# imazen/codec-eval

Hardware: AMD Instinct MI355X
Metric: metric MP/s (SSIMULACRA2+DSSIM+Butteraugli) at 1/2/4/8 GPU; HBM-roofline % (higher is better)
Workload: dtype f32

## Files before the change

### codec-eval_amd/csrc/butteraugli.hip

```cpp
#include <algorithm>
#include <cmath>
#include <cstdlib>
#include <type_traits>

#include "ba_front_geom.h"
#include "ba_slot_order.h"
#include "ce_internal.h"

namespace {

constexpr int TPB = 256;
constexpr int PSY = 10;
enum { UHF0 = 0, UHF1, HF0, HF1, MF0, MF1, MF2, LF0, LF1, LF2 };

struct blur_kernel {
    int len;
    float k[40];
    float lo[16], hi[16];
};

#define BA_XY                                                           \
    const uint32_t x = blockIdx.x * 64 + (threadIdx.x & 63);            \
    const uint32_t y = blockIdx.y * 4 + (threadIdx.x >> 6);             \
    if (x >= g.w || y >= g.h) return;                                   \
// ... 476 lines not shown
                float v[BW_OUT + LEN - 1];
#pragma unroll
                for (int j = 0; j < BW_OUT + LEN - 1; j++) v[j] = tile[(ly + j) * TW + c];
#pragma unroll
                for (int o = 0; o < BW_OUT; o++) {
                    float sum = 0.0f;
#pragma unroll
                    for (int j = 0; j < LEN; j++) sum = blur_tap(sum, v[o + j], bk.k[j]);
                    res[q][part][o] = sum * border_scale<LEN>(bk, gy0 + o, (int)g.h, inv_wsum);
                }
            }
        }
        if (HV && q + 1 < NP) {
            stash();
            __syncthreads();
        }
    }
    if (!col_live) return;
    const size_t pl = g.plane;
#pragma unroll
    for (int part = 0; part < PARTS; part++) {
        const int gy0 = y0 + 32 * part + 8 * wv;
        if (gy0 >= (int)g.h) break;
        float *ps = psy + (size_t)slot * PSY * g.plane + (size_t)gy0 * g.pitch + gx;
#pragma unroll
        for (int o = 0; o < BW_OUT; o++) {
            if (gy0 + o >= (int)g.h) break;
            float *q = ps + (size_t)o * g.pitch;
            const size_t ao = (size_t)slot * 3 * pl + (size_t)(gy0 + o) * g.pitch + gx;
            if (EPI == EPI_LF) {
                const float *xs = xyb + (size_t)slot * 3 * pl + (size_t)(gy0 + o) * g.pitch + gx;
                const float lx = res[0][part][o], ly = res[1][part][o], lb = res[2][part][o];
                aux_out[ao] = xs[0] - lx;
                aux_out[ao + pl] = xs[pl] - ly;
                aux_out[ao + 2 * pl] = xs[2 * pl] - lb;
                const float xmul = 33.832837186260f, ymul = 14.458268100570f, bmul = 49.87984651440f, y_to_b_mul = -0.362267051518f;
                const float bb = __builtin_fmaf(y_to_b_mul, ly, lb);
                q[LF2 * pl] = bb * bmul;
                q[LF0 * pl] = lx * xmul;
                q[LF1 * pl] = ly * ymul;
            } else if (EPI == EPI_MF) {
                const float kRemoveMfRange = 0.29f, kAddMfRange = 0.1f;
                const float mf0 = res[0][part][o], mf1 = res[1][part][o];
                const float hf0 = tmp[ao] - mf0, hf1 = tmp[ao + pl] - mf1;
                q[MF0 * pl] = remove_range(kRemoveMfRange, mf0);
                q[MF1 * pl] = amplify_range(kAddMfRange, mf1);
                q[MF2 * pl] = res[2][part][o];
                const float suppress = 46.0f, sv = 0.653020556257f, one_minus_s = 1.0f - 0.653020556257f;
                const float scaler = __builtin_fmaf(suppress / __builtin_fmaf(hf1, hf1, suppress), one_minus_s, sv);
                aux_out[ao] = scaler * hf0;
                aux_out[ao + pl] = hf1;
            } else if (EPI == EPI_MASK) {
                aux_out[(size_t)slot * pl + (size_t)(gy0 + o) * g.pitch + gx] = res[0][part][o];
            } else {
                const float kRemoveHfRange = 1.5f, kAddHfRange = 0.132f, kRemoveUhfRange = 0.04f;
                const float kMaxclampHf = 28.4691806922f, kMaxclampUhf = 5.19175294647f, kMulYHf = 2.155f, kMulYUhf = 2.69313763794f;
                float hf0_out, uhf0_out, hf1_out, uhf1_out;
                {
                    const float hf = res[0][part][o];
                    const float uhf = tmp[ao] - hf;
                    hf0_out = remove_range(kRemoveHfRange, hf);
                    uhf0_out = remove_range(kRemoveUhfRange, uhf);
                    q[HF0 * pl] = hf0_out;
                    q[UHF0 * pl] = uhf0_out;
                }
                {
                    float hf = maximum_clamp(res[1][part][o], kMaxclampHf);
                    float uhf = tmp[ao + pl] - hf;
                    uhf = maximum_clamp(uhf, kMaxclampUhf);
                    uhf *= kMulYUhf;
                    uhf1_out = uhf;
                    q[UHF1 * pl] = uhf;
                    hf *= kMulYHf;
                    hf1_out = amplify_range(kAddHfRange, hf);
                    q[HF1 * pl] = hf1_out;
                }
                mask_in[(size_t)slot * pl + (size_t)(gy0 + o) * g.pitch + gx] = mask_pre_one(uhf0_out, hf0_out, uhf1_out, hf1_out);
            }
        }
    }
}

struct malta_params {
    float norm2_0gt1, norm2_0lt1, norm1;
};

struct mline {
    int n;
    signed char d[9][2];
};

__device__ constexpr mline MALTA_HF[16] = {
    {9, {{-4, 0}, {-3, 0}, {-2, 0}, {-1, 0}, {0, 0}, {1, 0}, {2, 0}, {3, 0}, {4, 0}}},
    {9, {{0, -4}, {0, -3}, {0, -2}, {0, -1}, {0, 0}, {0, 1}, {0, 2}, {0, 3}, {0, 4}}},
    {7, {{-3, -3}, {-2, -2}, {-1, -1}, {0, 0}, {1, 1}, {2, 2}, {3, 3}}},
    {7, {{3, -3}, {2, -2}, {1, -1}, {0, 0}, {-1, 1}, {-2, 2}, {-3, 3}}},
    {9, {{1, -4}, {1, -3}, {1, -2}, {0, -1}, {0, 0}, {0, 1}, {-1, 2}, {-1, 3}, {-1, 4}}},
    {9, {{-1, -4}, {-1, -3}, {-1, -2}, {0, -1}, {0, 0}, {0, 1}, {1, 2}, {1, 3}, {1, 4}}},
    {9, {{-4, -1}, {-3, -1}, {-2, -1}, {-1, 0}, {0, 0}, {1, 0}, {2, 1}, {3, 1}, {4, 1}}},
    {9, {{-4, 1}, {-3, 1}, {-2, 1}, {-1, 0}, {0, 0}, {1, 0}, {2, -1}, {3, -1}, {4, -1}}},
    {7, {{-2, -3}, {-1, -2}, {-1, -1}, {0, 0}, {1, 1}, {1, 2}, {2, 3}}},
    {7, {{2, -3}, {1, -2}, {1, -1}, {0, 0}, {-1, 1}, {-1, 2}, {-2, 3}}},
    {7, {{-3, -2}, {-2, -1}, {-1, -1}, {0, 0}, {1, 1}, {2, 1}, {3, 2}}},
    {7, {{3, -2}, {2, -1}, {1, -1}, {0, 0}, {-1, 1}, {-2, 1}, {-3, 2}}},
    {8, {{-4, 2}, {-3, 2}, {-2, 1}, {-1, 1}, {0, 0}, {1, 0}, {2, -1}, {3, -1}}},
    {8, {{-4, -2}, {-3, -2}, {-2, -1}, {-1, -1}, {0, 0}, {1, 0}, {2, 1}, {3, 1}}},
    {8, {{-2, -4}, {-2, -3}, {-1, -2}, {-1, -1}, {0, 0}, {0, 1}, {1, 2}, {1, 3}}},
    {8, {{2, -4}, {2, -3}, {1, -2}, {1, -1}, {0, 0}, {0, 1}, {-1, 2}, {-1, 3}}},
};
__device__ constexpr mline MALTA_LF[16] = {
    {5, {{-4, 0}, {-2, 0}, {0, 0}, {2, 0}, {4, 0}}},
    {5, {{0, -4}, {0, -2}, {0, 0}, {0, 2}, {0, 4}}},
    {5, {{-3, -3}, {-2, -2}, {0, 0}, {2, 2}, {3, 3}}},
    {5, {{3, -3}, {2, -2}, {0, 0}, {-2, 2}, {-3, 3}}},
    {5, {{1, -4}, {1, -2}, {0, 0}, {-1, 2}, {-1, 4}}},
    {5, {{-1, -4}, {-1, -2}, {0, 0}, {1, 2}, {1, 4}}},
    {5, {{-4, -1}, {-2, -1}, {0, 0}, {2, 1}, {4, 1}}},
    {5, {{-4, 1}, {-2, 1}, {0, 0}, {2, -1}, {4, -1}}},
    {5, {{-2, -3}, {-1, -2}, {0, 0}, {1, 2}, {2, 3}}},
    {5, {{2, -3}, {1, -2}, {0, 0}, {-1, 2}, {-2, 3}}},
    {5, {{-3, -2}, {-2, -1}, {0, 0}, {2, 1}, {3, 2}}},
    {5, {{3, -2}, {2, -1}, {0, 0}, {-2, 1}, {-3, 2}}},
    {5, {{-4, 2}, {-2, 1}, {0, 0}, {2, -1}, {4, -2}}},
    {5, {{-4, -2}, {-2, -1}, {0, 0}, {2, 1}, {4, 2}}},
    {5, {{-2, -4}, {-1, -2}, {0, 0}, {1, 2}, {2, 4}}},
    {5, {{2, -4}, {1, -2}, {0, 0}, {-1, 2}, {-2, 4}}},
};

constexpr int MT = 64, MH = 4, ML = MT + 2 * MH;

__device__ constexpr bool malta_line_descends(const mline &ln)
{
    for (int j = 1; j < ln.n; j++)
        if (ln.d[j][1] > ln.d[j - 1][1]) return false;
    return ln.d[0][1] != ln.d[ln.n - 1][1];
}
__device__ constexpr bool malta_line_monotone(const mline &ln)
{
    bool up = true, down = true;
    for (int j = 1; j < ln.n; j++) {
        if (ln.d[j][1] < ln.d[j - 1][1]) up = false;
        if (ln.d[j][1] > ln.d[j - 1][1]) down = false;
    }
    return up || down;
}
__device__ constexpr bool malta_tables_monotone()
{
    for (int k = 0; k < 16; k++)
        if (!malta_line_monotone(MALTA_HF[k]) || !malta_line_monotone(MALTA_LF[k])) return false;
    return true;
}
static_assert(malta_tables_monotone(), "the row-streaming Malta unit needs every line's rows to be visited in one direction");

struct malta_bands {
    malta_params p[2][3];
};

__device__ __forceinline__ void div2_shared_rcp(float a0, float a1, float b, float &q0, float &q1)
{
    const float r = ce_rcp_refined(b);
    q0 = ce_div_refined(a0, b, r);
    q1 = ce_div_refined(a1, b, r);
}

__device__ __forceinline__ float malta_pre_diff(float v0, float v1, const malta_params &mp)
{
    const float absval = 0.5f * (fabsf(v0) + fabsf(v1));
    const float diff = v0 - v1;
    float scaler, scaler2;
    div2_shared_rcp(mp.norm2_0gt1, mp.norm2_0lt1, mp.norm1 + absval, scaler, scaler2);
    const float r = scaler * diff;
    const float fabs0 = fabsf(v0), too_small = 0.55f * fabs0, too_big = 1.05f * fabs0;
    const bool neg = v0 < 0;
    const float u = neg ? -v1 : v1;
    const bool lo = u < too_small, hi = u > too_big;
    const float impact = scaler2 * (lo ? too_small - u : u - too_big);
    const float rn = r + ((neg == lo) ? -impact : impact);
    return (lo || hi) ? rn : r;
}

__device__ __forceinline__ float l2_asym_acc(float total, float val0, float val1, float vw_0gt1, float vw_0lt1)
{
    const float diff = val0 - val1;
    total = __builtin_fmaf(diff * diff, vw_0gt1, total);
    const float fabs0 = fabsf(val0);
    const float too_small = 0.4f * fabs0, too_big = fabs0;
    const float if_neg = val1 > -too_small ? val1 + too_small : (val1 < -too_big ? -val1 - too_big : 0.0f);
    const float if_pos = val1 < too_small ? too_small - val1 : (val1 > too_big ? val1 - too_big : 0.0f);
    const float v = val0 < 0.0f ? if_neg : if_pos;
    return __builtin_fmaf(vw_0lt1, v * v, total);
}

template <bool LF>
__device__ __forceinline__ void malta_rows_xy(const ba_f2 *__restrict__ base, ba_f2 (&acc)[2])
{
    ba_f2 sum[2][16];
    ba_f2 parked[2][16][9];
#pragma unroll
    for (int r = 0; r < 9; r++) {
        ba_f2 v[10];
        const float4 *row = reinterpret_cast<const float4 *>(base + r * ML);
#pragma unroll
        for (int q = 0; q < 5; q++) {
            const float4 t = row[q];
            v[2 * q] = ba_f2{t.x, t.y};
            v[2 * q + 1] = ba_f2{t.z, t.w};
        }
        const int dy = r - 4;
#pragma unroll
        for (int o = 0; o < 2; o++) {
#pragma unroll
            for (int k = 0; k < 16; k++) {
                const mline &ln = LF ? MALTA_LF[k] : MALTA_HF[k];
                if (!malta_line_descends(ln)) {
#pragma unroll
                    for (int j = 0; j < 9; j++)
                        if (j < ln.n && ln.d[j][1] == dy) {
                            const ba_f2 t = v[4 + o + ln.d[j][0]];
                            sum[o][k] = j == 0 ? t : sum[o][k] + t;
                        }
                } else if (dy == ln.d[0][1]) {
                    ba_f2 acc_k = {0.0f, 0.0f};
#pragma unroll
                    for (int j = 0; j < 9; j++)
                        if (j < ln.n) {
                            const ba_f2 t = ln.d[j][1] == dy ? v[4 + o + ln.d[j][0]] : parked[o][k][j];
                            acc_k = j == 0 ? t : acc_k + t;
                        }
                    sum[o][k] = acc_k;
                } else {
#pragma unroll
                    for (int j = 0; j < 9; j++)
                        if (j < ln.n && ln.d[j][1] == dy) parked[o][k][j] = v[4 + o + ln.d[j][0]];
                }
            }
        }
    }
#pragma unroll
    for (int o = 0; o < 2; o++) {
        ba_f2 ret = {0.0f, 0.0f};
#pragma unroll
        for (int k = 0; k < 16; k++) ret = __builtin_elementwise_fma(sum[o][k], sum[o][k], ret);
        acc[o] = acc[o] + ret;
    }
}

template <int MR, int NT, bool FINAL, bool STORE>
__global__ __launch_bounds__(NT, NT == 256 ? 3 : 4) void k_ba_malta_l2_xy(const float *__restrict__ psy, const uint32_t *__restrict__ pair_ref,
                                                           const float *__restrict__ blurred, const float *__restrict__ mask_vals,
                                                           float *__restrict__ diffmap, ce_plane_geom g, uint32_t max_refs,
                                                           malta_bands mb, const uint2 *__restrict__ work, uint32_t tiles_x,
                                                           const float *__restrict__ sub_map, ce_plane_geom gs, int has_sub,
                                                           float *__restrict__ blk_max, double *__restrict__ blk_sums, uint32_t n_blocks)
{
    constexpr int MLR = MR + 2 * MH, RSTEP = NT / 32;
    __shared__ __attribute__((aligned(16))) ba_f2 s[MLR * ML];
    __shared__ __attribute__((aligned(16))) ba_f2 s_acc[MR * MT];
    const uint2 wi = work[blockIdx.x];
    if (wi.x == ~0u) return;
    const uint32_t p = wi.y, bx = wi.x % tiles_x, by = wi.x / tiles_x;
    const int x0 = (int)bx * MT - MH, y0 = (int)by * MR - MH;
    const float *a = psy + (size_t)pair_ref[p] * PSY * g.plane;
    const float *b = psy + (size_t)(max_refs + p) * PSY * g.plane;
    const int tq = threadIdx.x & 31, ty = threadIdx.x >> 5;
    const float wmul[9] = {400.0f, 1.50815703118f, 0.0f, 2150.0f, 10.6195433239f, 16.2176043152f, 29.2353797994f, 0.844626970982f, 0.703646627719f};
    const float hf_asymmetry = 1.0f;
#pragma unroll
    for (int band = 0; band < 3; band++) {
        const malta_params mpx = mb.p[0][band], mpy = mb.p[1][band];
        const uint32_t plane0 = band == 0 ? UHF0 : band == 1 ? HF0 : MF0;
        const float *pax = a + (size_t)plane0 * g.plane, *pbx = b + (size_t)plane0 * g.plane;
        const float *pay = pax + g.plane, *pby = pbx + g.plane;
        for (int i = threadIdx.x; i < MLR * (ML / 4); i += NT) {
            const int ly = i / (ML / 4), lq = i % (ML / 4), gx = x0 + 4 * lq, gy = y0 + ly;
            float4 vax = make_float4(0.f, 0.f, 0.f, 0.f), vbx = vax, vay = vax, vby = vax;
            const bool in = gx >= 0 && gy >= 0 && gx < (int)g.pitch && gy < (int)g.h;
            if (in) {
                const size_t o = (size_t)gy * g.pitch + gx;
                vax = *reinterpret_cast<const float4 *>(pax + o);
                vbx = *reinterpret_cast<const float4 *>(pbx + o);
                vay = *reinterpret_cast<const float4 *>(pay + o);
                vby = *reinterpret_cast<const float4 *>(pby + o);
            }
            const bool i0 = in && gx < (int)g.w, i1 = in && gx + 1 < (int)g.w, i2 = in && gx + 2 < (int)g.w, i3 = in && gx + 3 < (int)g.w;
            float4 r01, r23;
            r01.x = i0 ? malta_pre_diff(vax.x, vbx.x, mpx) : 0.0f;
            r01.y = i0 ? malta_pre_diff(vay.x, vby.x, mpy) : 0.0f;
            r01.z = i1 ? malta_pre_diff(vax.y, vbx.y, mpx) : 0.0f;
            r01.w = i1 ? malta_pre_diff(vay.y, vby.y, mpy) : 0.0f;
            r23.x = i2 ? malta_pre_diff(vax.z, vbx.z, mpx) : 0.0f;
            r23.y = i2 ? malta_pre_diff(vay.z, vby.z, mpy) : 0.0f;
            r23.z = i3 ? malta_pre_diff(vax.w, vbx.w, mpx) : 0.0f;
            r23.w = i3 ? malta_pre_diff(vay.w, vby.w, mpy) : 0.0f;
            float4 *dst = reinterpret_cast<float4 *>(s + ly * ML + 4 * lq);
            dst[0] = r01;
            dst[1] = r23;
            if (band >= 1 && ly >= MH && ly < MH + MR && lq >= MH / 4 && lq < (MH + MT) / 4 && gy < (int)g.h) {
                float4 *pa = reinterpret_cast<float4 *>(s_acc + (ly - MH) * MT + 4 * lq - MH);
                float4 t01 = pa[0], t23 = pa[1];
                if (band == 1) {
                    const float gx_ = wmul[0] * hf_asymmetry * 0.8f, lx_ = wmul[0] / hf_asymmetry * 0.8f;
                    const float gy_ = wmul[1] * hf_asymmetry * 0.8f, ly_ = wmul[1] / hf_asymmetry * 0.8f;
                    if (i0) t01.x = l2_asym_acc(t01.x, vax.x, vbx.x, gx_, lx_), t01.y = l2_asym_acc(t01.y, vay.x, vby.x, gy_, ly_);
                    if (i1) t01.z = l2_asym_acc(t01.z, vax.y, vbx.y, gx_, lx_), t01.w = l2_asym_acc(t01.w, vay.y, vby.y, gy_, ly_);
                    if (i2) t23.x = l2_asym_acc(t23.x, vax.z, vbx.z, gx_, lx_), t23.y = l2_asym_acc(t23.y, vay.z, vby.z, gy_, ly_);
                    if (i3) t23.z = l2_asym_acc(t23.z, vax.w, vbx.w, gx_, lx_), t23.w = l2_asym_acc(t23.w, vay.w, vby.w, gy_, ly_);
                } else {
                    auto l2 = [](float total, float v0, float v1, float w) {
                        const float diff = v0 - v1;
                        return __builtin_fmaf(diff * diff, w, total);
                    };
                    if (i0) t01.x = l2(t01.x, vax.x, vbx.x, wmul[3]), t01.y = l2(t01.y, vay.x, vby.x, wmul[4]);
                    if (i1) t01.z = l2(t01.z, vax.y, vbx.y, wmul[3]), t01.w = l2(t01.w, vay.y, vby.y, wmul[4]);
                    if (i2) t23.x = l2(t23.x, vax.z, vbx.z, wmul[3]), t23.y = l2(t23.y, vay.z, vby.z, wmul[4]);
                    if (i3) t23.z = l2(t23.z, vax.w, vbx.w, wmul[3]), t23.w = l2(t23.w, vay.w, vby.w, wmul[4]);
                }
                pa[0] = t01;
                pa[1] = t23;
            }
        }
        __syncthreads();
#pragma unroll 1
        for (int sub = 0; sub < MR / RSTEP; sub++) {
            ba_f2 acc[2] = {{0.f, 0.f}, {0.f, 0.f}};
            const ba_f2 *base = s + (RSTEP * sub + ty) * ML + 2 * tq;
            if (band == 0)
                malta_rows_xy<false>(base, acc);
            else
                malta_rows_xy<true>(base, acc);
            float4 *pacc = reinterpret_cast<float4 *>(s_acc + (RSTEP * sub + ty) * MT + 2 * tq);
            float4 t = make_float4(0.f, 0.f, 0.f, 0.f);
            if (band != 0) t = *pacc;
            *pacc = make_float4(t.x + acc[0].x, t.y + acc[0].y, t.z + acc[1].x, t.w + acc[1].y);
        }
        __syncthreads();
    }
    float red_m = 0.0f;
    double red_s3 = 0.0, red_s6 = 0.0, red_s12 = 0.0;
#pragma unroll 1
    for (int sub = 0; sub < MR / RSTEP; sub++) {
    float dmap[2] = {0.0f, 0.0f};
#pragma unroll
    for (int r = 0; r < 2; r++) {
        const uint32_t x = bx * MT + 2 * tq + r, y = by * MR + RSTEP * sub + ty;
        if (x >= g.w || y >= g.h) continue;
        const size_t o = (size_t)y * g.pitch + x;
        const ba_f2 sums = s_acc[(RSTEP * sub + ty) * MT + 2 * tq + r];
        float acv[3], dcv[3];
#pragma unroll
        for (uint32_t c = 0; c < 3; c++) {
            float total = c == 0 ? sums.x : c == 1 ? sums.y : 0.0f;
            if (c == 2) {
                const float diff = a[(MF0 + c) * g.plane + o] - b[(MF0 + c) * g.plane + o];
                total = __builtin_fmaf(diff * diff, wmul[3 + c], total);
            }
            acv[c] = total;
            {
                const float diff = a[(LF0 + c) * g.plane + o] - b[(LF0 + c) * g.plane + o];
                dcv[c] = (diff * diff) * wmul[6 + c];
            }
        }
        const size_t rslot = pair_ref[p];
        const float maskval = mask_vals[(rslot * 2 + 0) * g.plane + o], dc_maskval = mask_vals[(rslot * 2 + 1) * g.plane + o];
        const float mdiff = blurred[rslot * g.plane + o] - blurred[((size_t)max_refs + p) * g.plane + o];
        float ac0 = acv[0], ac1 = acv[1], ac2 = acv[2];
        float dc0 = dcv[0], dc1 = dcv[1], dc2 = dcv[2];
        ac1 += 10.0f * mdiff * mdiff;
        const float xmul = 1.0f;
        ac0 *= xmul;
        dc0 *= xmul;
        const float mc_dc = dc0 * dc_maskval + dc1 * dc_maskval + dc2 * dc_maskval;
        const float mc_ac = ac0 * maskval + ac1 * maskval + ac2 * maskval;
        float d = sqrtf(mc_dc + mc_ac);
        if (!FINAL) {
            diffmap[(size_t)p * g.plane + o] = d;
            continue;
        }
        if (has_sub) {
            const float kHeuristicMixingValue = 0.3f, wgt = 0.5f;
            d *= 1.0f - kHeuristicMixingValue * wgt;
            d += wgt * sub_map[(size_t)p * gs.plane + (size_t)(y / 2) * gs.pitch + x / 2];
        }
        const double dd = d, d3 = dd * dd * dd, d6 = d3 * d3;
        red_s3 += d3;
        red_s6 += d6;
        red_s12 += d6 * d6;
        red_m = fmaxf(red_m, d);
        if (STORE) dmap[r] = d;
    }
    if constexpr (FINAL && STORE) {
        const uint32_t x = bx * MT + 2 * tq, y = by * MR + RSTEP * sub + ty;
        if (x < g.w && y < g.h)
            *reinterpret_cast<float2 *>(diffmap + (size_t)p * g.plane + (size_t)y * g.pitch + x) = make_float2(dmap[0], dmap[1]);
    }
    }
    if (FINAL) {
        __shared__ float s_max[NT / 64];
        __shared__ double s_sum[3][NT / 64];
#pragma unroll
        for (int off = 32; off > 0; off >>= 1) {
            red_m = fmaxf(red_m, __shfl_down(red_m, off, 64));
            red_s3 += __shfl_down(red_s3, off, 64);
            red_s6 += __shfl_down(red_s6, off, 64);
            red_s12 += __shfl_down(red_s12, off, 64);
        }
        const int wv = threadIdx.x >> 6;
        if ((threadIdx.x & 63) == 0) {
            s_max[wv] = red_m;
            s_sum[0][wv] = red_s3;
            s_sum[1][wv] = red_s6;
            s_sum[2][wv] = red_s12;
        }
        __syncthreads();
        if (threadIdx.x == 0) {
            float mm = s_max[0];
            double sa = 0, sb = 0, sc = 0;
            for (int k = 0; k < NT / 64; k++) {
                mm = fmaxf(mm, s_max[k]);
                sa += s_sum[0][k];
                sb += s_sum[1][k];
                sc += s_sum[2][k];
            }
            const size_t bi = (size_t)p * n_blocks + wi.x;
            blk_max[bi] = mm;
            blk_sums[bi * 3] = sa;
            blk_sums[bi * 3 + 1] = sb;
            blk_sums[bi * 3 + 2] = sc;
        }
    }
}


__device__ __forceinline__ void store_min3(float v, float &min0, float &min1, float &min2)
{
    const float a = fminf(min0, v), t = fmaxf(min0, v);
    const float b = fminf(min1, t), u = fmaxf(min1, t);
    min2 = fminf(min2, u);
    min1 = b;
    min0 = a;
}

__global__ __launch_bounds__(TPB) void k_ba_mask_vals(const float *__restrict__ blurred, float *__restrict__ vals, ce_plane_geom g)
{
    const uint32_t z = blockIdx.z;
    BA_XY;
    const float *from = blurred + (size_t)z * g.plane;
    const int X = (int)x, Y = (int)y, W = (int)g.w, H = (int)g.h, S = 3;
    const uint32_t pitch = g.pitch;
#define at(yy, xx) from[(size_t)(yy) * pitch + (xx)]
    const int xl = max(X - S, 0), xr = min(X + S, W - 1), yu = max(Y - S, 0), yd = min(Y + S, H - 1);
    const float c0 = at(Y, X);
    const float v_l = at(Y, xl), v_lu = at(yu, xl), v_ld = at(yd, xl), v_r = at(Y, xr), v_ru = at(yu, xr), v_rd = at(yd, xr),
                v_u = at(yu, X), v_d = at(yd, X);
    const bool hl = X >= S, hr = X < W - S, hu = Y >= S, hd = Y < H - S;
    const float INF = __builtin_inff();
    float min0 = c0, min1 = 2 * min0, min2 = min1;
    store_min3(hl ? v_l : INF, min0, min1, min2);
    store_min3(hl && hu ? v_lu : INF, min0, min1, min2);
    store_min3(hl && hd ? v_ld : INF, min0, min1, min2);
    store_min3(hr ? v_r : INF, min0, min1, min2);
    store_min3(hr && hu ? v_ru : INF, min0, min1, min2);
    store_min3(hr && hd ? v_rd : INF, min0, min1, min2);
    store_min3(hu ? v_u : INF, min0, min1, min2);
    store_min3(hd ? v_d : INF, min0, min1, min2);
    const float mask = 0.45f * min0 + 0.3f * min1 + 0.25f * min2;
#undef at
    const double kGlobalScale = 1.0 / (17.83 * 0.790799174);
    const double val = (double)mask;
    double c = 2.5485944793 / ((0.451936922203 * val) + 0.829591754942);
    double rv = kGlobalScale * (1.0 + c);
    vals[((size_t)z * 2 + 0) * g.plane + o] = (float)(rv * rv);
    c = 0.505054525019 / ((3.87449418804 * val) + 0.20025578522);
    rv = kGlobalScale * (1.0 + c);
    vals[((size_t)z * 2 + 1) * g.plane + o] = (float)(rv * rv);
}

__global__ __launch_bounds__(TPB) void k_ba_score(const float *__restrict__ blk_max, const double *__restrict__ blk_sums,
                                                  ce_dev_scores *__restrict__ scores, double *__restrict__ pnorm,
                                                  uint32_t n_blocks, uint32_t used_blocks, double npix)
{
    __shared__ float s_max[TPB];
    __shared__ double s_sum[3][TPB];
    const uint32_t p = blockIdx.x, t = threadIdx.x;
    float mx = 0.0f;
    double s[3] = {0, 0, 0};
    for (uint32_t k = t; k < used_blocks; k += TPB) {
        mx = fmaxf(mx, blk_max[(size_t)p * n_blocks + k]);
        for (int q = 0; q < 3; q++) s[q] += blk_sums[((size_t)p * n_blocks + k) * 3 + q];
    }
    s_max[t] = mx;
    for (int q = 0; q < 3; q++) s_sum[q][t] = s[q];
    __syncthreads();
    for (int off = TPB / 2; off > 0; off >>= 1) {
        if ((int)t < off) {
            s_max[t] = fmaxf(s_max[t], s_max[t + off]);
            for (int q = 0; q < 3; q++) s_sum[q][t] += s_sum[q][t + off];
        }
        __syncthreads();
    }
    if (t == 0) {
        scores[p].butteraugli = (double)s_max[0];
        const double opp = 1.0 / npix;
        pnorm[p] = (pow(opp * s_sum[0][0], 1.0 / 3.0) + pow(opp * s_sum[1][0], 1.0 / 6.0) + pow(opp * s_sum[2][0], 1.0 / 12.0)) / 3.0;
    }
}

constexpr uint32_t DIV_SWEEP_EXP_FIRST = 87u, DIV_SWEEP_EXP_SPAN = 132u;
__global__ __launch_bounds__(256) void k_div_sweep(uint64_t seed, uint64_t count, unsigned long long *out)
{
    unsigned long long bad = 0;
    for (uint64_t i = (uint64_t)blockIdx.x * blockDim.x + threadIdx.x; i < count; i += (uint64_t)gridDim.x * blockDim.x) {
        uint64_t x = (i + seed) * 0x9E3779B97F4A7C15ull;
        x = (x ^ (x >> 30)) * 0xBF58476D1CE4E5B9ull;
        x = (x ^ (x >> 27)) * 0x94D049BB133111EBull;
        x ^= x >> 31;
        const uint32_t mb = (uint32_t)x & 0x7fffffu, ma = (uint32_t)(x >> 23) & 0x7fffffu, m2 = (uint32_t)(x >> 41) & 0x7fffffu;
        const uint32_t eb = DIV_SWEEP_EXP_FIRST + (uint32_t)((x >> 17) % DIV_SWEEP_EXP_SPAN),
                       ea = DIV_SWEEP_EXP_FIRST + (uint32_t)((x >> 7) % DIV_SWEEP_EXP_SPAN),
                       e2 = DIV_SWEEP_EXP_FIRST + (uint32_t)((x >> 3) % DIV_SWEEP_EXP_SPAN);
        const float b = __uint_as_float((eb << 23) | mb | ((uint32_t)(x >> 61) & 1u) << 31);
        float a0 = __uint_as_float((ea << 23) | ma | ((uint32_t)(x >> 60) & 1u) << 31), a1 = __uint_as_float((e2 << 23) | m2);
        if ((x >> 50 & 1023u) == 0) a0 = 0.0f;
        float q0, q1;
        div2_shared_rcp(a0, a1, b, q0, q1);
        const float w0 = a0 / b, w1 = a1 / b;
        const bool in0 = a0 == 0.0f || (fabsf(w0) >= 1.17549435e-38f && fabsf(w0) <= 3.40282347e+38f);
        const bool in1 = fabsf(w1) >= 1.17549435e-38f && fabsf(w1) <= 3.40282347e+38f;
        bad += (in0 && __float_as_uint(q0) != __float_as_uint(w0)) + (in1 && __float_as_uint(q1) != __float_as_uint(w1));
        bad += in1 && __float_as_uint(ce_div_noscale(a1, b)) != __float_as_uint(w1);
    }
    if (bad) atomicAdd(out, bad);
}

blur_kernel make_kernel(float sigma)
{
    blur_kernel bk{};
    const float m = 2.25f;
    const double scaler = -1.0 / (2.0 * (double)sigma * (double)sigma);
    int diff = (int)(m * std::fabs(sigma));
    if (diff < 1) diff = 1;
    for (int i = -diff; i <= diff; i++) bk.k[i + diff] = (float)std::exp(scaler * i * i);
    bk.len = 2 * diff + 1;
    for (int d = 0; d < diff && d < 16; d++) {
        float lo = 0.0f, hi = 0.0f;
        for (int j = diff - d; j < bk.len; j++) lo += bk.k[j];
        for (int j = 0; j <= diff + d; j++) hi += bk.k[j];
        bk.lo[d] = 1.0f / lo;
        bk.hi[d] = 1.0f / hi;
    }
    return bk;
}

float inv_weight_sum(const blur_kernel &bk)
{
    float wsum = 0.0f;
    for (int j = 0; j < bk.len; j++) wsum += bk.k[j];
    return 1.0f / wsum;
}

malta_params make_malta(double w_0gt1, double w_0lt1, double norm1, bool lf)
{
    const double len = 3.75, mulli = lf ? 0.611612573796 : 0.39905817637;
    const float kWeight0 = 0.5f, kWeight1 = 0.33f;
    const double w_pre0gt1 = mulli * std::sqrt(kWeight0 * w_0gt1) / (len * 2 + 1);
    const double w_pre0lt1 = mulli * std::sqrt(kWeight1 * w_0lt1) / (len * 2 + 1);
    return malta_params{(float)(w_pre0gt1 * norm1), (float)(w_pre0lt1 * norm1), (float)norm1};
}

}

int ce_butteraugli_div_sweep(ce_ctx *ctx, uint64_t seed, uint64_t count, uint64_t *mismatches)
{
    unsigned long long *d = nullptr, h = 0;
    CE_HIP(ctx, hipMalloc(&d, sizeof(h)));
    CE_HIP(ctx, hipMemsetAsync(d, 0, sizeof(h), ctx->stream));
    CE_LAUNCH(ctx, "div_sweep", k_div_sweep, dim3(4096), dim3(256), 0, seed, count, d);
    CE_HIP(ctx, hipMemcpyAsync(&h, d, sizeof(h), hipMemcpyDeviceToHost, ctx->stream));
    CE_HIP(ctx, hipStreamSynchronize(ctx->stream));
    CE_HIP(ctx, hipFree(d));
    if (mismatches) *mismatches = h;
    return CE_OK;
}

static int ba_prepare(ce_batch *b)
{
    if (b->ba.engaged()) return CE_OK;
    ce_ctx *ctx = b->ctx;
    ce_ba_set B;
    auto set = [](ce_plane_geom &d, uint32_t w, uint32_t h) {
        d.w = w;
        d.h = h;
        d.pitch = (w + 31u) & ~31u;
        d.plane = (size_t)d.pitch * h;
    };
    set(B.lvl[0], b->w, b->h);
    set(B.lvl[1], (b->w + 1) / 2, (b->h + 1) / 2);
    B.levels = (B.lvl[1].w >= 8 && B.lvl[1].h >= 8) ? 2 : 1;
    const size_t slots = (size_t)b->max_refs + b->max_pairs, P = b->max_pairs, p0 = B.lvl[0].plane;
    int rc = CE_OK;
    for (int l = 0; l < B.levels && rc == CE_OK; l++) {
        rc = B.psy[l].alloc(ctx, slots * PSY * B.lvl[l].plane);
        if (l == 1 && rc == CE_OK) rc = B.diff[l].alloc(ctx, P * B.lvl[l].plane);
    }
    for (auto &p : B.s)
        if (rc == CE_OK) rc = p.alloc(ctx, slots * 3 * p0);
    for (int l = 0; l < B.levels && rc == CE_OK; l++) {
        rc = B.mask[l].alloc(ctx, slots * B.lvl[l].plane);
        if (rc == CE_OK) rc = B.mask_vals[l].alloc(ctx, (size_t)b->max_refs * 2 * B.lvl[l].plane);
    }
    B.blocks = ((B.lvl[0].w + 63) / 64) * ((B.lvl[0].h + 3) / 4);
    if (rc == CE_OK) rc = B.blk_max.alloc(ctx, P * B.blocks);
    if (rc == CE_OK) rc = B.blk_sums.alloc(ctx, P * B.blocks * 3);
    if (rc == CE_OK) rc = B.pnorm.alloc(ctx, P);
    if (rc != CE_OK) return rc;
    b->ba = std::move(B);
    return CE_OK;
}

int ce_launch_butteraugli(ce_batch *b, const uint8_t *d_refs, uint32_t n_refs_used, uint32_t n_pairs, float intensity_target,
                          bool store_map)
{
    ce_ctx *ctx = b->ctx;
    int rc = ba_prepare(b);
    if (rc != CE_OK) return rc;
    if (store_map && !b->ba.map && b->ba.map.alloc((ce_ctx *)nullptr, (size_t)b->max_pairs * b->ba.lvl[0].plane) != CE_OK) {
        ctx->err = "out of device memory for the Butteraugli diffmaps";
        return CE_ERR_BACKEND;
    }
    const uint32_t n_slots = n_refs_used + n_pairs, mr = b->max_refs;
    const bool cached = b->refs.reuse(CE_REF_BUTTERAUGLI, d_refs, n_refs_used, ce_ref_param_f32(intensity_target));
    const uint32_t z0 = cached ? n_refs_used : 0, nz = n_slots - z0;
    const blur_kernel k12 = make_kernel(1.2f), kLf = make_kernel(7.15593339443f), kHf = make_kernel(3.22489901262f),
                      kUhf = make_kernel(1.56416327805f), kMask = make_kernel(2.7f);
    float sw = 0.0f;
    for (int j = 0; j < 5; j++) sw += k12.k[j];
    const float sc = 1.0f / sw, w0 = k12.k[2] * sc, w1 = k12.k[3] * sc, w2 = k12.k[4] * sc;
    const double hf_asymmetry = 1.0;
    const malta_params mUhfY = make_malta(1.10039032555 * hf_asymmetry, 1.10039032555 / hf_asymmetry, 71.7800275169, false);
    const malta_params mUhfX = make_malta(173.5 * hf_asymmetry, 173.5 / hf_asymmetry, 5.0, false);
    const malta_params mHfY = make_malta(18.7237414387 * std::sqrt(hf_asymmetry), 18.7237414387 / std::sqrt(hf_asymmetry), 4498534.45232, true);
    const malta_params mHfX = make_malta(6923.99476109 * std::sqrt(hf_asymmetry), 6923.99476109 / std::sqrt(hf_asymmetry), 8051.15833247, true);
    const malta_params mMfY = make_malta(37.0819870399, 37.0819870399, 130262059.556, true);
    const malta_params mMfX = make_malta(8246.75321353, 8246.75321353, 1009002.70582, true);

    const bool two_streams = b->ba.levels == 2 && !ctx->prof_serial && (double)n_pairs * b->w * b->h <= 4e6;
    hipStream_t s_main = CE_STREAM(ctx), s_half = s_main;
    if (two_streams) {
        if (!b->ba.half.stream) {
            ce_ba_half half;
            if (!(half.stream = ce_ctx_aux_stream(ctx, ce_ctx::AUX_BA_HALF))) return CE_ERR_BACKEND;
            if ((rc = half.ev_fork.create(ctx)) != CE_OK || (rc = half.ev_join.create(ctx)) != CE_OK) return rc;
            const size_t slots = (size_t)b->max_refs + b->max_pairs;
            for (auto &p : half.s)
                if ((rc = p.alloc(ctx, slots * 3 * b->ba.lvl[1].plane)) != CE_OK) return rc;
            b->ba.half = std::move(half);
        }
        s_half = b->ba.half.stream;
        CE_HIP(ctx, hipEventRecord(b->ba.half.ev_fork, s_main));
        CE_HIP(ctx, hipStreamWaitEvent(s_half, b->ba.half.ev_fork, 0));
    }
    static const uint32_t order_min = [] {
        const char *e = std::getenv("CE_BA_SLOT_ORDER_MIN");
        return e ? (uint32_t)std::atol(e) : ba_slot_order_min;
    }();
    static const uint32_t order_kernels = [] {
        const char *e = std::getenv("CE_BA_SLOT_ORDER_KERNELS");
        return e ? (uint32_t)std::atol(e) : 63u;
    }();
    uint32_t final_tiles = 0;
    for (int l = b->ba.levels - 1; l >= 0; l--) {
        const ce_plane_geom &d = b->ba.lvl[l], &g = d;
        const dim3 gx((d.w + 63) / 64, (d.h + 3) / 4, 1);
        auto G = [&](uint32_t z) { return dim3(gx.x, gx.y, z); };
        hipStream_t st = l == 1 ? s_half : s_main;
        const ce_dev<float> *scr = (two_streams && l == 1) ? b->ba.half.s : b->ba.s;
        float *psy = b->ba.psy[l], *sA = scr[0], *sC = scr[2];
        const plane_sel s3{3, 0, 3};
        auto SG = [&](uint32_t tile_w, uint32_t tile_h, uint32_t planes, uint32_t kernel_bit) {
            return ba_slot_grid_make((d.w + tile_w - 1) / tile_w, (d.h + tile_h - 1) / tile_h, planes, nz, z0,
                                     (order_kernels & kernel_bit) ? order_min : ~0u);
        };
        auto SB = [](const ba_slot_grid &s) {
            const ba_slot_dims3 dims = ba_slot_dims(s);
            return dim3(dims.x, dims.y, dims.z);
        };
        const ba_slot_grid sg_front = SG(FT, FT, 1, 1), sg_h33 = SG(256, 8 * BH_TILES, 3, 2), sg_vlf = SG(64, 32, 1, 4),
                           sg_mf = SG(64, 32, 1, 8), sg_hf = SG(64, 32, 1, 16), sg_mask = SG(64, 32, 1, 32);
        for (const ba_slot_grid &s : {sg_front, sg_h33, sg_vlf, sg_mf, sg_hf, sg_mask})
            if (ba_slot_dims(s).y > ba_slot_grid_yz_max || ba_slot_dims(s).z > ba_slot_grid_yz_max) {
                ctx->err = "Butteraugli batch too large for one launch";
                return CE_ERR_BACKEND;
            }
        const dim3 ft = SB(sg_front);
        const ce_plane_geom &gfull = b->ba.lvl[0];
        if (b->linear) {
            const float *none = nullptr;
            if (l == 0)
                CE_LAUNCH_ON(ctx, st, "ba_front_lin", (k_ba_front<false, float>), ft, dim3(TPB), 0, d_refs, b->d_tests, none, none, g, sC, g,
                             w0, w1, w2, intensity_target, b->img_bytes, n_refs_used, mr, sg_front);
            else
                CE_LAUNCH_ON(ctx, st, "ba_front_half_lin", (k_ba_front<true, float>), ft, dim3(TPB), 0, d_refs, b->d_tests, none, none, gfull,
                             sC, g, w0, w1, w2, intensity_target, b->img_bytes, n_refs_used, mr, sg_front);
        } else if (b->depth[0]) {
            const float *lr = b->deep_lut[0][0], *lt = b->deep_lut[0][1];
            if (l == 0)
                CE_LAUNCH_ON(ctx, st, "ba_front_u16", (k_ba_front<false, uint16_t>), ft, dim3(TPB), 0, d_refs, b->d_tests, lr, lt, g, sC, g,
                             w0, w1, w2, intensity_target, b->img_bytes, n_refs_used, mr, sg_front);
            else
                CE_LAUNCH_ON(ctx, st, "ba_front_half_u16", (k_ba_front<true, uint16_t>), ft, dim3(TPB), 0, d_refs, b->d_tests, lr, lt, gfull,
                             sC, g, w0, w1, w2, intensity_target, b->img_bytes, n_refs_used, mr, sg_front);
        } else if (l == 0) {
            CE_LAUNCH_ON(ctx, st, "ba_front_u8", (k_ba_front<false, uint8_t>), ft, dim3(TPB), 0, d_refs, b->d_tests, ctx->d_lut_ssim2,
                         ctx->d_lut_ssim2, g, sC, g, w0, w1, w2, intensity_target, b->img_bytes, n_refs_used, mr, sg_front);
        } else {
            CE_LAUNCH_ON(ctx, st, "ba_front_half", (k_ba_front<true, uint8_t>), ft, dim3(TPB), 0, d_refs, b->d_tests, ctx->d_lut_ssim2,
                         ctx->d_lut_ssim2, gfull, sC, g, w0, w1, w2, intensity_target, b->img_bytes, n_refs_used, mr, sg_front);
        }
        {
            if (kLf.len != 33 || kHf.len != 15 || kUhf.len != 7) {
                ctx->err = "unexpected blur kernel length";
                return CE_ERR_BACKEND;
            }
            float *sB = scr[1];
            CE_LAUNCH_ON(ctx, st, "ba_blur_h33", k_ba_blur_h<33>, SB(sg_h33), dim3(TPB), 0, (const float *)sC, sA, g, s3, s3, kLf, inv_weight_sum(kLf),
                      n_refs_used, mr, 1, sg_h33);
            CE_LAUNCH_ON(ctx, st, "ba_blur_v_lf", (k_ba_blur_v_split<33, EPI_LF, false, 32>), SB(sg_vlf), dim3(TPB), 0, (const float *)sA,
                         (const float *)sC, psy, g, kLf, inv_weight_sum(kLf), n_refs_used, mr, sg_vlf, (float *)nullptr, sB);
            CE_LAUNCH_ON(ctx, st, "ba_blur_hv_mf", (k_ba_blur_v_split<15, EPI_MF, true, 32>), SB(sg_mf), dim3(TPB), 0, (const float *)sB,
                         (const float *)nullptr, psy, g, kHf, inv_weight_sum(kHf), n_refs_used, mr, sg_mf, (float *)nullptr, sA);
            CE_LAUNCH_ON(ctx, st, "ba_blur_hv_hf", (k_ba_blur_v_split<7, EPI_HF, true, 32>), SB(sg_hf), dim3(TPB), 0, (const float *)sA,
                         (const float *)nullptr, psy, g, kUhf, inv_weight_sum(kUhf), n_refs_used, mr, sg_hf, sB, (float *)nullptr);
        }

        {
            if (kMask.len != 13) {
                ctx->err = "unexpected blur kernel length";
                return CE_ERR_BACKEND;
            }
            CE_LAUNCH_ON(ctx, st, "ba_blur_hv_mask", (k_ba_blur_v_split<13, EPI_MASK, true, 32>), SB(sg_mask), dim3(TPB), 0, (const float *)scr[1],
                      (const float *)nullptr, psy, g, kMask, inv_weight_sum(kMask), n_refs_used, mr, sg_mask, (float *)nullptr, b->ba.mask[l]);
        }
        if (!cached)
            CE_LAUNCH_ON(ctx, st, "ba_mask_vals", k_ba_mask_vals, G(n_refs_used), dim3(TPB), 0, (const float *)b->ba.mask[l], b->ba.mask_vals[l], g);

        malta_bands mb;
        mb.p[0][0] = mUhfX; mb.p[0][1] = mHfX; mb.p[0][2] = mMfX;
        mb.p[1][0] = mUhfY; mb.p[1][1] = mHfY; mb.p[1][2] = mMfY;
        const uint32_t tiles_x = (d.w + MT - 1) / MT, tiles_y = (d.h + 31) / 32;
        if ((rc = ce_build_xcd_list(b, n_pairs, ce_xcd_keys{1, tiles_x * tiles_y, 1}, &b->ba.work[l])) != CE_OK) return rc;
        const bool has_sub = b->ba.levels == 2;
        const ce_plane_geom &gsub = b->ba.lvl[has_sub ? 1 : 0];
#define CE_MALTA_ARGS(FINAL, STORE)                                                                                                \
    psy, b->d_pair_ref, (const float *)b->ba.mask[l], (const float *)b->ba.mask_vals[l],                                               \
        STORE ? b->ba.map : FINAL ? (float *)nullptr : b->ba.diff[1], g, mr, mb, (const uint2 *)b->ba.work[l].d, tiles_x,             \
        FINAL ? (const float *)b->ba.diff[1] : (const float *)nullptr, gsub, has_sub ? 1 : 0, b->ba.blk_max, b->ba.blk_sums, b->ba.blocks
        const dim3 gmalta(b->ba.work[l].len);
        if (l == 0) {
            final_tiles = tiles_x * tiles_y;
            if (two_streams) CE_HIP(ctx, hipStreamWaitEvent(s_main, b->ba.half.ev_join, 0));
            if (store_map)
                CE_LAUNCH_ON(ctx, st, "ba_malta_l2_map", (k_ba_malta_l2_xy<32, 256, true, true>), gmalta, dim3(256), 0, CE_MALTA_ARGS(true, true));
            else
                CE_LAUNCH_ON(ctx, st, "ba_malta_l2", (k_ba_malta_l2_xy<32, 256, true, false>), gmalta, dim3(256), 0, CE_MALTA_ARGS(true, false));
        } else {
            CE_LAUNCH_ON(ctx, st, "ba_malta_l2", (k_ba_malta_l2_xy<32, 256, false, false>), gmalta, dim3(256), 0, CE_MALTA_ARGS(false, false));
            if (two_streams) CE_HIP(ctx, hipEventRecord(b->ba.half.ev_join, s_half));
        }
#undef CE_MALTA_ARGS
    }
    const auto &d0 = b->ba.lvl[0];
    CE_LAUNCH(ctx, "ba_score", k_ba_score, dim3(n_pairs), dim3(TPB), 0, b->ba.blk_max, b->ba.blk_sums, b->d_scores, b->ba.pnorm,
              b->ba.blocks, final_tiles, (double)d0.w * (double)d0.h);
    CE_HIP(ctx, hipGetLastError());
    if (!cached) b->refs.built(CE_REF_BUTTERAUGLI, d_refs, n_refs_used, ce_ref_param_f32(intensity_target));
    return CE_OK;
}

int ce_butteraugli_read_maps(ce_batch *b, uint32_t first, uint32_t count, uint32_t block, float *out)
{
    return ce_read_map_cells(b, "ba_block_max", b->ba.map, b->ba.lvl[0], first, count, block, false, b->ba.cells, out);
}
```

Baseline: 21440.

## Vectorize Malta pre-diff over x/y pairs and batch tile loads before compute

Packs the X and Y channel Malta parameters into paired two-lane vectors so the pre-diff division and refinement run as packed float2 math. It also restructures the shared-memory fill: per-thread quad metadata is precomputed into bitmasks, all global float4 loads for a thread are issued before any compute, and a compile-time interior path drops the bounds checks for tiles fully inside the image. This is meant to cut VALU instruction count and raise memory-level parallelism in the fill phase, at the cost of more live registers (NI sets of four float4 values), which may reduce occupancy.

Measured after the change: 21650, median of 6. 1.01x the previous value.

```diff
diff --git a/codec-eval_amd/csrc/butteraugli.hip b/codec-eval_amd/csrc/butteraugli.hip
--- a/codec-eval_amd/csrc/butteraugli.hip
+++ b/codec-eval_amd/csrc/butteraugli.hip
@@ -652,31 +652,45 @@
 }
 static_assert(malta_tables_monotone(), "the row-streaming Malta unit needs every line's rows to be visited in one direction");
 
+struct malta_params_xy {
+    ba_f2 norm2_0gt1, norm2_0lt1, norm1;
+};
 struct malta_bands {
-    malta_params p[2][3];
+    malta_params_xy p[3];
 };
-
-__device__ __forceinline__ void div2_shared_rcp(float a0, float a1, float b, float &q0, float &q1)
-{
-    const float r = ce_rcp_refined(b);
-    q0 = ce_div_refined(a0, b, r);
-    q1 = ce_div_refined(a1, b, r);
-}
-
-__device__ __forceinline__ float malta_pre_diff(float v0, float v1, const malta_params &mp)
-{
-    const float absval = 0.5f * (fabsf(v0) + fabsf(v1));
-    const float diff = v0 - v1;
-    float scaler, scaler2;
-    div2_shared_rcp(mp.norm2_0gt1, mp.norm2_0lt1, mp.norm1 + absval, scaler, scaler2);
-    const float r = scaler * diff;
-    const float fabs0 = fabsf(v0), too_small = 0.55f * fabs0, too_big = 1.05f * fabs0;
-    const bool neg = v0 < 0;
-    const float u = neg ? -v1 : v1;
-    const bool lo = u < too_small, hi = u > too_big;
-    const float impact = scaler2 * (lo ? too_small - u : u - too_big);
-    const float rn = r + ((neg == lo) ? -impact : impact);
-    return (lo || hi) ? rn : r;
+__host__ inline malta_params_xy malta_pair(const malta_params &x, const malta_params &y)
+{
+    return malta_params_xy{ba_f2{x.norm2_0gt1, y.norm2_0gt1}, ba_f2{x.norm2_0lt1, y.norm2_0lt1}, ba_f2{x.norm1, y.norm1}};
+}
+
+__device__ __forceinline__ ba_f2 rcp_refined_xy(ba_f2 b)
+{
+    const ba_f2 r0 = {__builtin_amdgcn_rcpf(b.x), __builtin_amdgcn_rcpf(b.y)};
+    return __builtin_elementwise_fma(__builtin_elementwise_fma(-b, r0, ba_f2{1.0f, 1.0f}), r0, r0);
+}
+__device__ __forceinline__ ba_f2 div_refined_xy(ba_f2 a, ba_f2 b, ba_f2 r)
+{
+    ba_f2 q = a * r;
+    q = __builtin_elementwise_fma(__builtin_elementwise_fma(-b, q, a), r, q);
+    return __builtin_elementwise_fma(__builtin_elementwise_fma(-b, q, a), r, q);
+}
+
+__device__ __forceinline__ ba_f2 malta_pre_diff_xy(ba_f2 v0, ba_f2 v1, const malta_params_xy &mp)
+{
+    const ba_f2 fabs0 = __builtin_elementwise_abs(v0);
+    const ba_f2 absval = ba_f2{0.5f, 0.5f} * (fabs0 + __builtin_elementwise_abs(v1));
+    const ba_f2 diff = v0 - v1;
+    const ba_f2 den = mp.norm1 + absval, rden = rcp_refined_xy(den);
+    const ba_f2 scaler = div_refined_xy(mp.norm2_0gt1, den, rden), scaler2 = div_refined_xy(mp.norm2_0lt1, den, rden);
+    const ba_f2 r = scaler * diff;
+    const ba_f2 too_small = ba_f2{0.55f, 0.55f} * fabs0, too_big = ba_f2{1.05f, 1.05f} * fabs0;
+    const bool negx = v0.x < 0, negy = v0.y < 0;
+    const ba_f2 u = {negx ? -v1.x : v1.x, negy ? -v1.y : v1.y};
+    const bool lox = u.x < too_small.x, loy = u.y < too_small.y, hix = u.x > too_big.x, hiy = u.y > too_big.y;
+    const ba_f2 below = too_small - u, above = u - too_big;
+    const ba_f2 impact = scaler2 * ba_f2{lox ? below.x : above.x, loy ? below.y : above.y};
+    const ba_f2 rn = r + ba_f2{(negx == lox) ? -impact.x : impact.x, (negy == loy) ? -impact.y : impact.y};
+    return ba_f2{(lox || hix) ? rn.x : r.x, (loy || hiy) ? rn.y : r.y};
 }
 
 __device__ __forceinline__ float l2_asym_acc(float total, float val0, float val1, float vw_0gt1, float vw_0lt1)
@@ -765,60 +779,87 @@
     const int tq = threadIdx.x & 31, ty = threadIdx.x >> 5;
     const float wmul[9] = {400.0f, 1.50815703118f, 0.0f, 2150.0f, 10.6195433239f, 16.2176043152f, 29.2353797994f, 0.844626970982f, 0.703646627719f};
     const float hf_asymmetry = 1.0f;
+    constexpr int NQ = MLR * (ML / 4), NI = (NQ + NT - 1) / NT;
+    static_assert(MH > 0, "the tile's last quad must hold no own pixel");
+    constexpr uint32_t FQ_LOAD = 16, FQ_OWN = 32;
+    const bool interior = x0 >= 0 && y0 >= 0 && x0 + ML <= (int)g.w && y0 + MLR <= (int)g.h;
 #pragma unroll
     for (int band = 0; band < 3; band++) {
-        const malta_params mpx = mb.p[0][band], mpy = mb.p[1][band];
+        const malta_params_xy mp = mb.p[band];
         const uint32_t plane0 = band == 0 ? UHF0 : band == 1 ? HF0 : MF0;
         const float *pax = a + (size_t)plane0 * g.plane, *pbx = b + (size_t)plane0 * g.plane;
         const float *pay = pax + g.plane, *pby = pbx + g.plane;
-        for (int i = threadIdx.x; i < MLR * (ML / 4); i += NT) {
-            const int ly = i / (ML / 4), lq = i % (ML / 4), gx = x0 + 4 * lq, gy = y0 + ly;
-            float4 vax = make_float4(0.f, 0.f, 0.f, 0.f), vbx = vax, vay = vax, vby = vax;
+        uint32_t fq[NI];
+        int tid = threadIdx.x;
+        asm volatile("" : "+v"(tid));
+#pragma unroll
+        for (int k = 0; k < NI; k++) {
+            const int i = min(tid + k * NT, NQ - 1), ly = i / (ML / 4), lq = i % (ML / 4), gx = x0 + 4 * lq, gy = y0 + ly;
             const bool in = gx >= 0 && gy >= 0 && gx < (int)g.pitch && gy < (int)g.h;
-            if (in) {
+            const bool own = ly >= MH && ly < MH + MR && lq >= MH / 4 && lq < (MH + MT) / 4 && gy < (int)g.h;
+            uint32_t m = (uint32_t)ly << 8 | (uint32_t)lq << 16 | (own ? FQ_OWN : 0u) | (in ? FQ_LOAD : 0u);
+#pragma unroll
+            for (int j = 0; j < 4; j++) m |= (in && gx + j < (int)g.w) ? 1u << j : 0u;
+            fq[k] = m;
+        }
+        auto fill = [&](auto interior_c) {
+            constexpr bool INTERIOR = decltype(interior_c)::value;
+            float4 vax[NI], vbx[NI], vay[NI], vby[NI];
+            auto load = [&](int k) {
+                const bool in = INTERIOR || (fq[k] & FQ_LOAD);
+                const int gy = in ? y0 + (int)(fq[k] >> 8 & 0xff) : 0, gx = in ? x0 + 4 * (int)(fq[k] >> 16) : 0;
                 const size_t o = (size_t)gy * g.pitch + gx;
-                vax = *reinterpret_cast<const float4 *>(pax + o);
-                vbx = *reinterpret_cast<const float4 *>(pbx + o);
-                vay = *reinterpret_cast<const float4 *>(pay + o);
-                vby = *reinterpret_cast<const float4 *>(pby + o);
-            }
-            const bool i0 = in && gx < (int)g.w, i1 = in && gx + 1 < (int)g.w, i2 = in && gx + 2 < (int)g.w, i3 = in && gx + 3 < (int)g.w;
-            float4 r01, r23;
-            r01.x = i0 ? malta_pre_diff(vax.x, vbx.x, mpx) : 0.0f;
-            r01.y = i0 ? malta_pre_diff(vay.x, vby.x, mpy) : 0.0f;
-            r01.z = i1 ? malta_pre_diff(vax.y, vbx.y, mpx) : 0.0f;
-            r01.w = i1 ? malta_pre_diff(vay.y, vby.y, mpy) : 0.0f;
-            r23.x = i2 ? malta_pre_diff(vax.z, vbx.z, mpx) : 0.0f;
-            r23.y = i2 ? malta_pre_diff(vay.z, vby.z, mpy) : 0.0f;
-            r23.z = i3 ? malta_pre_diff(vax.w, vbx.w, mpx) : 0.0f;
-            r23.w = i3 ? malta_pre_diff(vay.w, vby.w, mpy) : 0.0f;
-            float4 *dst = reinterpret_cast<float4 *>(s + ly * ML + 4 * lq);
-            dst[0] = r01;
-            dst[1] = r23;
-            if (band >= 1 && ly >= MH && ly < MH + MR && lq >= MH / 4 && lq < (MH + MT) / 4 && gy < (int)g.h) {
-                float4 *pa = reinterpret_cast<float4 *>(s_acc + (ly - MH) * MT + 4 * lq - MH);
-                float4 t01 = pa[0], t23 = pa[1];
-                if (band == 1) {
-                    const float gx_ = wmul[0] * hf_asymmetry * 0.8f, lx_ = wmul[0] / hf_asymmetry * 0.8f;
-                    const float gy_ = wmul[1] * hf_asymmetry * 0.8f, ly_ = wmul[1] / hf_asymmetry * 0.8f;
-                    if (i0) t01.x = l2_asym_acc(t01.x, vax.x, vbx.x, gx_, lx_), t01.y = l2_asym_acc(t01.y, vay.x, vby.x, gy_, ly_);
-                    if (i1) t01.z = l2_asym_acc(t01.z, vax.y, vbx.y, gx_, lx_), t01.w = l2_asym_acc(t01.w, vay.y, vby.y, gy_, ly_);
-                    if (i2) t23.x = l2_asym_acc(t23.x, vax.z, vbx.z, gx_, lx_), t23.y = l2_asym_acc(t23.y, vay.z, vby.z, gy_, ly_);
-                    if (i3) t23.z = l2_asym_acc(t23.z, vax.w, vbx.w, gx_, lx_), t23.w = l2_asym_acc(t23.w, vay.w, vby.w, gy_, ly_);
-                } else {
-                    auto l2 = [](float total, float v0, float v1, float w) {
-                        const float diff = v0 - v1;
-                        return __builtin_fmaf(diff * diff, w, total);
-                    };
-                    if (i0) t01.x = l2(t01.x, vax.x, vbx.x, wmul[3]), t01.y = l2(t01.y, vay.x, vby.x, wmul[4]);
-                    if (i1) t01.z = l2(t01.z, vax.y, vbx.y, wmul[3]), t01.w = l2(t01.w, vay.y, vby.y, wmul[4]);
-                    if (i2) t23.x = l2(t23.x, vax.z, vbx.z, wmul[3]), t23.y = l2(t23.y, vay.z, vby.z, wmul[4]);
-                    if (i3) t23.z = l2(t23.z, vax.w, vbx.w, wmul[3]), t23.w = l2(t23.w, vay.w, vby.w, wmul[4]);
+                vax[k] = *reinterpret_cast<const float4 *>(pax + o);
+                vbx[k] = *reinterpret_cast<const float4 *>(pbx + o);
+                vay[k] = *reinterpret_cast<const float4 *>(pay + o);
+                vby[k] = *reinterpret_cast<const float4 *>(pby + o);
+            };
+            auto scale = [&](int k) {
+                const int ly = fq[k] >> 8 & 0xff, lq = fq[k] >> 16;
+                const bool i0 = INTERIOR || (fq[k] & 1), i1 = INTERIOR || (fq[k] & 2), i2 = INTERIOR || (fq[k] & 4), i3 = INTERIOR || (fq[k] & 8);
+                const ba_f2 zero = {0.0f, 0.0f};
+                const ba_f2 d0 = malta_pre_diff_xy(ba_f2{vax[k].x, vay[k].x}, ba_f2{vbx[k].x, vby[k].x}, mp);
+                const ba_f2 d1 = malta_pre_diff_xy(ba_f2{vax[k].y, vay[k].y}, ba_f2{vbx[k].y, vby[k].y}, mp);
+                const ba_f2 d2 = malta_pre_diff_xy(ba_f2{vax[k].z, vay[k].z}, ba_f2{vbx[k].z, vby[k].z}, mp);
+                const ba_f2 d3 = malta_pre_diff_xy(ba_f2{vax[k].w, vay[k].w}, ba_f2{vbx[k].w, vby[k].w}, mp);
+                const ba_f2 e0 = i0 ? d0 : zero, e1 = i1 ? d1 : zero, e2 = i2 ? d2 : zero, e3 = i3 ? d3 : zero;
+                float4 *dst = reinterpret_cast<float4 *>(s + ly * ML + 4 * lq);
+                dst[0] = make_float4(e0.x, e0.y, e1.x, e1.y);
+                dst[1] = make_float4(e2.x, e2.y, e3.x, e3.y);
+                if (band >= 1 && (fq[k] & FQ_OWN)) {
+                    const float4 ax = vax[k], bx_ = vbx[k], ay = vay[k], by_ = vby[k];
+                    float4 *pa = reinterpret_cast<float4 *>(s_acc + (ly - MH) * MT + 4 * lq - MH);
+                    float4 t01 = pa[0], t23 = pa[1];
+                    if (band == 1) {
+                        const float gx_ = wmul[0] * hf_asymmetry * 0.8f, lx_ = wmul[0] / hf_asymmetry * 0.8f;
+                        const float gy_ = wmul[1] * hf_asymmetry * 0.8f, ly_ = wmul[1] / hf_asymmetry * 0.8f;
+                        if (i0) t01.x = l2_asym_acc(t01.x, ax.x, bx_.x, gx_, lx_), t01.y = l2_asym_acc(t01.y, ay.x, by_.x, gy_, ly_);
+                        if (i1) t01.z = l2_asym_acc(t01.z, ax.y, bx_.y, gx_, lx_), t01.w = l2_asym_acc(t01.w, ay.y, by_.y, gy_, ly_);
+                        if (i2) t23.x = l2_asym_acc(t23.x, ax.z, bx_.z, gx_, lx_), t23.y = l2_asym_acc(t23.y, ay.z, by_.z, gy_, ly_);
+                        if (i3) t23.z = l2_asym_acc(t23.z, ax.w, bx_.w, gx_, lx_), t23.w = l2_asym_acc(t23.w, ay.w, by_.w, gy_, ly_);
+                    } else {
+                        auto l2 = [](float total, float v0, float v1, float w) {
+                            const float diff = v0 - v1;
+                            return __builtin_fmaf(diff * diff, w, total);
+                        };
+                        if (i0) t01.x = l2(t01.x, ax.x, bx_.x, wmul[3]), t01.y = l2(t01.y, ay.x, by_.x, wmul[4]);
+                        if (i1) t01.z = l2(t01.z, ax.y, bx_.y, wmul[3]), t01.w = l2(t01.w, ay.y, by_.y, wmul[4]);
+                        if (i2) t23.x = l2(t23.x, ax.z, bx_.z, wmul[3]), t23.y = l2(t23.y, ay.z, by_.z, wmul[4]);
+                        if (i3) t23.z = l2(t23.z, ax.w, bx_.w, wmul[3]), t23.w = l2(t23.w, ay.w, by_.w, wmul[4]);
+                    }
+                    pa[0] = t01;
+                    pa[1] = t23;
                 }
-                pa[0] = t01;
-                pa[1] = t23;
-            }
-        }
+            };
+#pragma unroll
+            for (int k = 0; k < NI; k++) load(k);
+#pragma unroll
+            for (int k = 0; k < NI; k++) scale(k);
+        };
+        if (interior)
+            fill(std::true_type{});
+        else
+            fill(std::false_type{});
         __syncthreads();
 #pragma unroll 1
         for (int sub = 0; sub < MR / RSTEP; sub++) {
@@ -1021,8 +1062,8 @@
         const float b = __uint_as_float((eb << 23) | mb | ((uint32_t)(x >> 61) & 1u) << 31);
         float a0 = __uint_as_float((ea << 23) | ma | ((uint32_t)(x >> 60) & 1u) << 31), a1 = __uint_as_float((e2 << 23) | m2);
         if ((x >> 50 & 1023u) == 0) a0 = 0.0f;
-        float q0, q1;
-        div2_shared_rcp(a0, a1, b, q0, q1);
+        const ba_f2 bb = {b, b}, q01 = div_refined_xy(ba_f2{a0, a1}, bb, rcp_refined_xy(bb));
+        const float q0 = q01.x, q1 = q01.y;
         const float w0 = a0 / b, w1 = a1 / b;
         const bool in0 = a0 == 0.0f || (fabsf(w0) >= 1.17549435e-38f && fabsf(w0) <= 3.40282347e+38f);
         const bool in1 = fabsf(w1) >= 1.17549435e-38f && fabsf(w1) <= 3.40282347e+38f;
@@ -1244,8 +1285,7 @@
             CE_LAUNCH_ON(ctx, st, "ba_mask_vals", k_ba_mask_vals, G(n_refs_used), dim3(TPB), 0, (const float *)b->ba.mask[l], b->ba.mask_vals[l], g);
 
         malta_bands mb;
-        mb.p[0][0] = mUhfX; mb.p[0][1] = mHfX; mb.p[0][2] = mMfX;
-        mb.p[1][0] = mUhfY; mb.p[1][1] = mHfY; mb.p[1][2] = mMfY;
+        mb.p[0] = malta_pair(mUhfX, mUhfY); mb.p[1] = malta_pair(mHfX, mHfY); mb.p[2] = malta_pair(mMfX, mMfY);
         const uint32_t tiles_x = (d.w + MT - 1) / MT, tiles_y = (d.h + 31) / 32;
         if ((rc = ce_build_xcd_list(b, n_pairs, ce_xcd_keys{1, tiles_x * tiles_y, 1}, &b->ba.work[l])) != CE_OK) return rc;
         const bool has_sub = b->ba.levels == 2;
```
